# jhauret/vibravox

Measured on AMD Instinct MI355X. Metric: EBEN train-step audio-seconds/sec (gen+disc), higher is better.
Workload: dtype bf16

## Files before the change

vibravox_amd/csrc/bl_dw.hip:

```cpp
#include "common.h"

#include <cstdlib>

namespace eben {

typedef float f32x16 __attribute__((ext_vector_type(16)));
typedef __bf16 bf16x8 __attribute__((ext_vector_type(8)));
typedef short s16x4 __attribute__((ext_vector_type(4)));
typedef short s16x8 __attribute__((ext_vector_type(8)));
typedef unsigned u32x4 __attribute__((ext_vector_type(4)));

#ifndef EBEN_BLDW_DBG
#define EBEN_BLDW_DBG 0
#endif
#ifndef EBEN_BLDW_PIPE_FENCE
#define EBEN_BLDW_PIPE_FENCE 1
#endif
#ifdef EBEN_BLDW_STAMP
__device__ unsigned long long bldw_stamp[8192 * 8];
#define BLDW_T(v) const unsigned long long v = __builtin_amdgcn_s_memtime()
#endif
constexpr int BLDW_BKT = 64;
constexpr int BLDW_TS = 68;
constexpr int BLDW_RS_MAX = 132;
static int bldw_row_stride(int xneed) { int rs = xneed <= 4 ? 4 : xneed; while ((rs & 15) != 4) ++rs; return rs > BLDW_RS_MAX ? BLDW_RS_MAX : rs; }

struct BlDwArgs {
  const u32x4* ah; const u32x4* xh;
  float* slabs;
  int B, G, Mg, Cg, MgB, CgB, CBa, CBx, La, Lx;
  int S, d, k, pad, amin;
  int NQW;
  int has_bias, nnt, nmt, nsplit, nct, nchunks, XR, xneed;
  int dense, c_in_g, c_out_g, row_stride;
  int RS;
  int xw;
  long long slab_stride;
};

template <unsigned STEP4 = 64u>
__device__ __forceinline__ bf16x8 bl_tr_frag(unsigned addr) {
  typedef __attribute__((address_space(3))) s16x4* lds4_t;
  const s16x4 r0 = __builtin_amdgcn_ds_read_tr16_b64_v4i16((lds4_t)(size_t)(addr));
  const s16x4 r1 = __builtin_amdgcn_ds_read_tr16_b64_v4i16((lds4_t)(size_t)(addr + STEP4));
  const s16x8 v = {r0[0], r0[1], r0[2], r0[3], r1[0], r1[1], r1[2], r1[3]};
  return __builtin_bit_cast(bf16x8, v);
}

__device__ u32x4 bl_zero_unit = {0u, 0u, 0u, 0u};

__device__ __forceinline__ void bl_dma_piece(const u32x4* src, unsigned dst) {
  asm volatile("s_mov_b32 m0, %1\n\ts_nop 0\n\tglobal_load_lds_dwordx4 %0, off" :: "v"(src), "s"(dst) : "memory");
}

constexpr int BLDW_XC_S = 4;
template <int FM, int FN, bool XC = false, int WN = 2>
__device__ __forceinline__ void bl_dw_body(const BlDwArgs& P, unsigned bid, unsigned nblk) {
  constexpr int BM = 64 * FM, BMB = BM / 8, BNQ = 4 * WN * FN, BKT = BLDW_BKT, TS = BLDW_TS, NW = 2 * WN;
  const int RS = P.RS;
  extern __shared__ __attribute__((aligned(16))) u32x4 smem_bldw[];
  typedef __attribute__((address_space(3))) void* lds_t;
  const int tid = threadIdx.x, lane = tid & 63;
  const int wave = __builtin_amdgcn_readfirstlane(tid >> 6);
  const int wm = wave / WN, wn = wave % WN;

  unsigned id = xcd_remap(bid, nblk);
  const int z = __builtin_amdgcn_readfirstlane(id % P.nsplit); id /= P.nsplit;
  const int nti = __builtin_amdgcn_readfirstlane(id % P.nnt); id /= P.nnt;
  const int mt = __builtin_amdgcn_readfirstlane(id % P.nmt);
  const int g = __builtin_amdgcn_readfirstlane(id / P.nmt);

  const int q0 = nti * BNQ;
  int cb_lo = q0 / P.k;
  if (cb_lo > P.CgB - 1) cb_lo = P.CgB - 1;
  int qlast = q0 + BNQ < P.NQW ? q0 + BNQ : P.NQW;
  int cb_hi = (qlast - 1) / P.k;
  if (cb_hi < cb_lo) cb_hi = cb_lo;
  const int xrows = (cb_hi - cb_lo + 1) * (XC ? 1 : P.S);

  const int a_units = BMB * TS, buf_units = a_units + P.XR * RS;
  for (int i = tid; i < BLDW_TS; i += 64 * NW) smem_bldw[i] = u32x4{0x00003f80u, 0u, 0u, 0u};
  const unsigned lds0 = (unsigned)(unsigned long long)(lds_t)smem_bldw;
  const unsigned ones_addr = lds0, buf_addr = lds0 + BLDW_TS * 16;

  const int G4 = lane >> 4, js = (lane & 15) >> 2, qs = lane & 3;
  const int koff = 8 * (G4 >> 1) + js;
  unsigned aoff[FM], boff[FN];
  bool bconst[FN];
#pragma unroll
  for (int i = 0; i < FM; ++i) {
    const int bundle = (wm * FM + i) * 4 + 2 * (G4 & 1) + (qs >> 1);
    aoff[i] = (unsigned)((bundle * TS + koff) * 16 + 8 * (qs & 1));
  }
#pragma unroll
  for (int f = 0; f < FN; ++f) {
    const int q = q0 + 4 * (wn * FN + f) + 2 * (G4 & 1) + (qs >> 1);
    if (q < P.NQW) {
      const int cb = q / P.k, j = q - cb * P.k;
      const int off = j * P.d - P.pad;
      if (XC) {
        boff[f] = (unsigned)(a_units * 16 + ((cb - cb_lo) * RS + (off - P.amin * BLDW_XC_S) + koff * BLDW_XC_S) * 16 + 8 * (qs & 1));
      } else {
        int a = off / P.S;
        if (off < 0 && a * P.S != off) --a;
        const int p = off - a * P.S;
        const int row = (cb - cb_lo) * P.S + p;
        boff[f] = (unsigned)(a_units * 16 + (row * RS + (a - P.amin) + koff) * 16 + 8 * (qs & 1));
      }
      bconst[f] = false;
    } else {
      boff[f] = (unsigned)(koff * 16 + 8 * (qs & 1));
      bconst[f] = true;
    }
  }

  f32x16 acc[FM][FN];
#pragma unroll
  for (int i = 0; i < FM; ++i)
#pragma unroll
    for (int f = 0; f < FN; ++f)
#pragma unroll
      for (int r = 0; r < 16; ++r) acc[i][f][r] = 0.f;

  const u32x4* zero = &bl_zero_unit;
  constexpr int AR = (BMB + NW - 1) / NW;
  long long arow[AR];
#pragma unroll
  for (int i = 0; i < AR; ++i) {
    int bundle = g * P.MgB + mt * BMB + wave + NW * i;
    if (bundle > P.CBa - 1) bundle = P.CBa - 1;
    arow[i] = mt * BMB + wave + NW * i < P.MgB ? (long long)bundle * P.La : -1;
  }
  constexpr int XW = 4;
  const bool x_regs = XC || P.XR <= NW * XW;
  long long xoff[XW];
  int xlane[XW];
  unsigned xdst[XW];
  bool xact[XW];
  const int npr = XC ? (P.xw + 63) / 64 : 1;
#pragma unroll
  for (int i = 0; i < XW; ++i) {
    const int xr = wave + NW * i;
    if (XC) {
      const int row = xr / npr, pc = xr - row * npr;
      int cb = cb_lo + row;
      if (cb > P.CgB - 1) cb = P.CgB - 1;
      xoff[i] = ((long long)g * P.CgB + cb) * P.Lx;
      xlane[i] = P.amin * BLDW_XC_S + 64 * pc + lane;
      xdst[i] = (unsigned)((a_units + row * RS + 64 * pc) * 16);
      xact[i] = xr < xrows * npr && 64 * pc + lane < P.xw;
    } else {
      const int cbl = xr / P.S, p = xr - cbl * P.S;
      int cb = cb_lo + cbl;
      if (cb > P.CgB - 1) cb = P.CgB - 1;
      xoff[i] = ((long long)g * P.CgB + cb) * P.Lx;
      xlane[i] = (P.amin + lane) * P.S + p;
      xdst[i] = (unsigned)((a_units + xr * RS) * 16);
      xact[i] = true;
    }
  }
  const long long a_item = (long long)P.CBa * P.La, x_item = (long long)P.CBx * P.Lx;
  auto issue = [&](int b, int t0, int bsel) {
    const unsigned dst = buf_addr + (unsigned)(bsel * buf_units * 16);
    const u32x4* ab = P.ah + (long long)b * a_item + t0 + lane;
    const bool a_ok = t0 + lane < P.La;
#pragma unroll
    for (int i = 0; i < AR; ++i) {
      const int r = wave + NW * i;
      if (r < BMB && !(EBEN_BLDW_DBG & 1)) bl_dma_piece((a_ok && arow[i] >= 0) ? ab + arow[i] : zero, __builtin_amdgcn_readfirstlane(dst + (unsigned)(r * TS * 16)));
    }
    const u32x4* xb = P.xh + (long long)b * x_item;
    if (EBEN_BLDW_DBG & 2) return;
    if (XC) {
      const int ts = t0 * BLDW_XC_S;
#pragma unroll
      for (int i = 0; i < XW; ++i)
        if (wave + NW * i < xrows * npr) {
          const int pos0 = ts + xlane[i];
          if (xact[i]) bl_dma_piece((unsigned)pos0 < (unsigned)P.Lx ? xb + xoff[i] + pos0 : zero, __builtin_amdgcn_readfirstlane(dst + xdst[i]));
        }
      return;
    }
    if (x_regs) {
      const int ts = t0 * P.S;
#pragma unroll
      for (int i = 0; i < XW; ++i)
        if (wave + NW * i < xrows) {
          const u32x4* row = xb + xoff[i];
          const int pos0 = ts + xlane[i];
          const unsigned rdst = dst + xdst[i];
          bl_dma_piece((unsigned)pos0 < (unsigned)P.Lx ? row + pos0 : zero, __builtin_amdgcn_readfirstlane(rdst));
          if (64 + lane < P.xneed) {
            const int pos1 = pos0 + 64 * P.S;
            bl_dma_piece((unsigned)pos1 < (unsigned)P.Lx ? row + pos1 : zero, __builtin_amdgcn_readfirstlane(rdst + (unsigned)(64 * 16)));
          }
        }
      return;
    }
    for (int xr = wave; xr < xrows; xr += NW) {
      const int cbl = xr / P.S, p = xr - cbl * P.S;
      int cb = cb_lo + cbl;
      if (cb > P.CgB - 1) cb = P.CgB - 1;
      const u32x4* row = xb + ((long long)g * P.CgB + cb) * P.Lx;
      const unsigned rdst = dst + (unsigned)((a_units + xr * RS) * 16);
      const int pos0 = (t0 + P.amin + lane) * P.S + p;
      bl_dma_piece((pos0 >= 0 && pos0 < P.Lx) ? row + pos0 : zero, __builtin_amdgcn_readfirstlane(rdst));
      if (64 + lane < P.xneed) {
        const int pos1 = pos0 + 64 * P.S;
        bl_dma_piece((pos1 >= 0 && pos1 < P.Lx) ? row + pos1 : zero, __builtin_amdgcn_readfirstlane(rdst + (unsigned)(64 * 16)));
      }
    }
  };
  const int dq_b = P.nsplit / P.nct, dq_t = P.nsplit - dq_b * P.nct;
  int qb = z / P.nct, qt = z - qb * P.nct;

  int bsel = 0;
  auto advance = [&]() {
    qb += dq_b; qt += dq_t;
    if (qt >= P.nct) { qt -= P.nct; ++qb; }
  };
  if (z < P.nchunks) { issue(qb, qt * BKT, 0); advance(); }
#ifdef EBEN_BLDW_STAMP
  unsigned long long st_wait = 0, st_bar = 0, st_issue = 0, st_mma = 0, st_n = 0;
  const unsigned long long st_begin = __builtin_amdgcn_s_memtime();
#endif
  for (int q = z; q < P.nchunks; q += P.nsplit) {
#ifdef EBEN_BLDW_STAMP
    BLDW_T(ta);
#endif
    asm volatile("s_waitcnt vmcnt(0)" ::: "memory");
#ifdef EBEN_BLDW_STAMP
    BLDW_T(tb);
#endif
    __syncthreads();
#ifdef EBEN_BLDW_STAMP
    BLDW_T(tc);
#endif
    if (q + P.nsplit < P.nchunks) { issue(qb, qt * BKT, bsel ^ 1); advance(); }
#ifdef EBEN_BLDW_STAMP
    BLDW_T(td);
#endif
    const unsigned base = buf_addr + (unsigned)(bsel * buf_units * 16);
    constexpr unsigned BSTEP4 = XC ? 64u * BLDW_XC_S : 64u;
    bf16x8 av[2][FM], bv[2][FN];
#pragma unroll
    for (int i = 0; i < FM; ++i) av[0][i] = bl_tr_frag(base + aoff[i]);
#pragma unroll
    for (int f = 0; f < FN; ++f) bv[0][f] = bl_tr_frag<BSTEP4>(bconst[f] ? ones_addr + boff[f] : base + boff[f]);
#pragma unroll
    for (int ks = 0; ks < BKT / 16; ++ks) {
      const int cur = ks & 1, nxt = cur ^ 1;
      if (ks + 1 < BKT / 16) {
#pragma unroll
        for (int i = 0; i < FM; ++i) av[nxt][i] = bl_tr_frag(base + aoff[i] + (unsigned)((ks + 1) * 256));
#pragma unroll
        for (int f = 0; f < FN; ++f)
          bv[nxt][f] = bl_tr_frag<BSTEP4>(bconst[f] ? ones_addr + boff[f] : base + boff[f] + (unsigned)((ks + 1) * 4 * BSTEP4));
      }
#pragma unroll
      for (int i = 0; i < FM; ++i)
#pragma unroll
        for (int f = 0; f < FN; ++f) {
          if (EBEN_BLDW_DBG & 4) acc[i][f][0] += __builtin_bit_cast(float, __builtin_bit_cast(u32x4, av[cur][i])[0] ^ __builtin_bit_cast(u32x4, bv[cur][f])[1]);
          else acc[i][f] = __builtin_amdgcn_mfma_f32_32x32x16_bf16(av[cur][i], bv[cur][f], acc[i][f], 0, 0, 0);
        }
#if EBEN_BLDW_PIPE_FENCE
      __builtin_amdgcn_sched_barrier(0);
#endif
    }
    bsel ^= 1;
#ifdef EBEN_BLDW_STAMP
    { BLDW_T(te); st_wait += tb - ta; st_bar += tc - tb; st_issue += td - tc; st_mma += te - td; ++st_n; }
#endif
  }
#ifdef EBEN_BLDW_STAMP
  if (tid == 0 && bid < 8192u) {
    unsigned long long* o = bldw_stamp + bid * 8;
    o[0] = st_wait; o[1] = st_bar; o[2] = st_issue; o[3] = st_mma; o[4] = st_n; o[5] = __builtin_amdgcn_s_memtime() - st_begin;
  }
#endif

  float* slab = P.slabs + (long long)z * P.slab_stride;
  const int m_base = mt * BM + wm * FM * 32 + 4 * (lane >> 5);
#pragma unroll
  for (int f = 0; f < FN; ++f) {
    const int nl = lane & 31;
    const int q = q0 + 4 * (wn * FN + f) + (nl >> 3), e = nl & 7;
    long long col = -1;
    int cgrp = -1;
    if (!P.dense) {
      if (q < P.NQW || (q == P.NQW && e == 0 && P.has_bias)) col = 8LL * q + e;
    } else if (q < P.NQW) {
      const int cb = q / P.k, j = q - cb * P.k, c = 8 * cb + e;
      cgrp = c / P.c_in_g;
      col = (long long)(c - cgrp * P.c_in_g) * P.k + j;
    } else if (q == P.NQW && e == 0 && P.has_bias) {
      col = (long long)P.c_in_g * P.k;
    }
    if (col < 0) continue;
#pragma unroll
    for (int i = 0; i < FM; ++i)
#pragma unroll
      for (int r = 0; r < 16; ++r) {
        const int m = m_base + i * 32 + (r & 3) + 8 * (r >> 2);
        if (m >= P.Mg) continue;
        if (P.dense && cgrp >= 0 && m / P.c_out_g != cgrp) continue;
        if (!(EBEN_BLDW_DBG & 8) || acc[i][f][r] == 12345.f) slab[((long long)g * P.Mg + m) * P.row_stride + col] = acc[i][f][r];
      }
  }
}

template <int FM, int FN, bool XC = false, int WN = 2>
__global__ __launch_bounds__(128 * WN, 2) void bl_dw_kernel(const BlDwArgs P) { bl_dw_body<FM, FN, XC, WN>(P, blockIdx.x, gridDim.x); }

constexpr int BLDW_MULTI = 4;
struct BlDwTable {
  int n;
  unsigned first[BLDW_MULTI + 1];
  BlDwArgs job[BLDW_MULTI];
};
template <int FM, int FN>
__global__ __launch_bounds__(256, 2) void bl_dw_multi_kernel(const BlDwTable T) {
  int j = 0;
#pragma unroll 1
  while (j + 1 < T.n && blockIdx.x >= T.first[j + 1]) ++j;
  j = __builtin_amdgcn_readfirstlane(j);
  bl_dw_body<FM, FN>(T.job[j], blockIdx.x - T.first[j], T.first[j + 1] - T.first[j]);
}

struct BlDwPlan {
  int ok, G, Mg, Cg, MgB, CgB, dense, FM, FN, nmt, nnt, NQW, nct, nchunks, nsplit, XR, amin, row_stride, perm_k, xneed, RS, xc, xw, wide;
  size_t lds_bytes;
  long long slab_stride;
};

static int bldw_floordiv(int a, int b) { int q = a / b; if ((a % b != 0) && ((a < 0) != (b < 0))) --q; return q; }

static void make_bldw_plan(const Canon& c, BlDwPlan* p) {
  p->ok = 0;
  if (!c.bl || c.reflect || c.np != 1) return;
  p->G = c.g; p->Mg = c.Cout / c.g; p->Cg = c.Cin / c.g; p->dense = 0;
  if ((p->Mg & 7) || (p->Cg & 7)) { p->dense = 1; p->G = 1; p->Mg = c.Cout; p->Cg = c.Cin; }
  if ((p->Mg & 7) || (p->Cg & 7)) return;
  p->MgB = p->Mg / 8; p->CgB = p->Cg / 8;
  p->amin = bldw_floordiv(-c.pl, c.s);
  const int amax = bldw_floordiv((c.k - 1) * c.d - c.pl, c.s);
  if (amax - p->amin > 60 || c.s > 8) return;
  p->FM = (p->Mg > 64 && round_up(p->Mg, 128) == round_up(p->Mg, 64)) ? 2 : 1;
  p->NQW = p->CgB * c.k;
  static const int fn_max = getenv("EBEN_BLDW_FN") ? atoi(getenv("EBEN_BLDW_FN")) : 4;
  p->FN = (fn_max >= 4 && (c.k >= 16 || p->NQW >= 256)) ? 4 : p->NQW + 1 > 8 ? 2 : 1;
  static const int fn3_thin = getenv("EBEN_BLDW_FN3_THIN") ? atoi(getenv("EBEN_BLDW_FN3_THIN")) : 1;
  if (fn3_thin && p->FN == 2 && ceil_div(p->NQW + 1, 24) < ceil_div(p->NQW + 1, 16)) p->FN = 3;
  static const int fn3 = getenv("EBEN_BLDW_FN3") ? atoi(getenv("EBEN_BLDW_FN3")) : 1;
  if (fn3 && p->FN == 4 && p->FM == 2) {
    const int t4 = ceil_div(p->NQW + 1, 32) * ceil_div(p->Mg, 64 * p->FM) * p->G, t3 = ceil_div(p->NQW + 1, 24) * ceil_div(p->Mg, 64 * p->FM) * p->G;
    if (fn3 == 2 || (t4 <= 512 && t4 > 256 && t3 <= 512)) p->FN = 3;
  }
  static const int wide_on = getenv("EBEN_BLDW_WIDE") ? atoi(getenv("EBEN_BLDW_WIDE")) : 1;
  p->wide = (wide_on && p->FM == 2 && p->FN >= 3 && p->NQW + 1 >= 48 && c.s == BLDW_XC_S && c.d == 1) ? 1 : 0;
  if (p->wide) p->FN = 3;
  static const int xc_on = getenv("EBEN_BLDW_XC") ? atoi(getenv("EBEN_BLDW_XC")) : 1;
  p->nmt = ceil_div(p->Mg, 64 * p->FM);
  p->xneed = BLDW_BKT + amax - p->amin + 1;
  for (;;) {
    const int BNQ = (p->wide ? 16 : 8) * p->FN;
    p->nnt = ceil_div(p->NQW + 1, BNQ);
    int ncb = (BNQ - 1) / c.k + 2;
    if (ncb > p->CgB) ncb = p->CgB;
    p->XR = ncb * c.s;
    p->RS = bldw_row_stride(p->xneed);
    p->xc = 0; p->xw = 0;
    if (xc_on && c.s == BLDW_XC_S && c.d == 1 && p->FN >= 3) {
      const int xw = p->xneed * c.s;
      if (ncb * ceil_div(xw, 64) <= (p->wide ? 32 : 16)) {
        p->xc = 1; p->xw = xw; p->XR = ncb;
        p->RS = xw + 1;
      }
    }
    if (!p->wide || p->xc) break;
    p->wide = 0;
  }
  p->lds_bytes = 16ull * (BLDW_TS + 2ull * ((64 * p->FM / 8) * BLDW_TS + (unsigned long long)p->XR * p->RS));
  if (p->lds_bytes > 160 * 1024) return;
  p->nct = ceil_div(c.Lout, BLDW_BKT);
  p->nchunks = c.B * p->nct;
  const int tiles = p->nnt * p->nmt * p->G;
  static const int cus = getenv("EBEN_BLDW_CUS") ? atoi(getenv("EBEN_BLDW_CUS")) : 256;
  const int per_cu = p->wide ? 1 : (int)(160 * 1024 / p->lds_bytes) < 1 ? 1 : (int)(160 * 1024 / p->lds_bytes);
  const int slots = cus * (per_cu > 4 ? 4 : per_cu);
  const double macs = (double)c.B * c.Lout * (double)c.Cout * (c.Cin / c.g) * c.k;
  const double t_all = 2.0 * macs / 1.0e15;
  const double slab_bytes = 4.0 * (double)c.Cout * ((c.Cin / c.g) * c.k + 1);
  int ns = 1;
  double best = 1e30;
  for (int cand = 1; cand <= 256 && cand <= p->nchunks; ++cand) {
    const long long blocks = (long long)tiles * cand;
    const double rounds = (double)((blocks + slots - 1) / slots);
    const double t = rounds * (t_all * slots / blocks) + 2.0 * cand * slab_bytes / 2.0e12 + (cand > 1 ? slab_bytes / 2.0e12 + 5e-6 : 0.0);
    if (t < best * 0.97) { best = t; ns = cand; }
  }
  static const int force_ns = getenv("EBEN_BLDW_NSPLIT") ? atoi(getenv("EBEN_BLDW_NSPLIT")) : 0;
  if (force_ns > 0 && force_ns <= p->nchunks) ns = force_ns;
  p->nsplit = ns;
  if (p->dense) { p->row_stride = (c.Cin / c.g) * c.k + 1; p->perm_k = 0; }
  else { p->row_stride = p->Cg * c.k + 1; p->perm_k = c.k; }
  p->slab_stride = (long long)c.Cout * p->row_stride;
  p->ok = 1;
}

template <int FM, int FN, bool XC = false, int WN = 2>
static int launch_bldw(const BlDwArgs& a, const BlDwPlan& p, hipStream_t st) {
  static LdsAttrOnce attr_once;
  auto kern = bl_dw_kernel<FM, FN, XC, WN>;
  {
    const hipError_t e = lds_attr_once(attr_once, reinterpret_cast<const void*>(kern));
    if (e != hipSuccess) return hip_fail(e, "hipFuncSetAttribute(bl_dw)");
  }
  const long long nb = (long long)p.nnt * p.nmt * p.G * p.nsplit;
  hipLaunchKernelGGL(kern, dim3((unsigned)nb), dim3(128 * WN), p.lds_bytes, st, a);
  EBEN_CHECK_LAUNCH("bl_dw_kernel");
  return EBEN_OK;
}

struct BlDwVariant { int FM, FN, XC, WN, grouped; };
static BlDwVariant bldw_variant(const BlDwPlan& p) {
  if (p.wide) return BlDwVariant{2, 3, 1, 4, 0};
  return BlDwVariant{p.FM, p.FN, p.xc, 2, p.xc ? 0 : 1};
}

static int launch_bldw_variant(const BlDwVariant& v, const BlDwArgs& a, const BlDwPlan& p, hipStream_t st) {
  if (v.WN == 4) return launch_bldw<2, 3, true, 4>(a, p, st);
  if (v.XC) return v.FM == 2 ? (v.FN == 4 ? launch_bldw<2, 4, true>(a, p, st) : launch_bldw<2, 3, true>(a, p, st))
                             : (v.FN == 4 ? launch_bldw<1, 4, true>(a, p, st) : launch_bldw<1, 3, true>(a, p, st));
  if (v.FM == 2) return v.FN == 4 ? launch_bldw<2, 4>(a, p, st) : v.FN == 3 ? launch_bldw<2, 3>(a, p, st) : v.FN == 2 ? launch_bldw<2, 2>(a, p, st) : launch_bldw<2, 1>(a, p, st);
  return v.FN == 4 ? launch_bldw<1, 4>(a, p, st) : v.FN == 3 ? launch_bldw<1, 3>(a, p, st) : v.FN == 2 ? launch_bldw<1, 2>(a, p, st) : launch_bldw<1, 1>(a, p, st);
}

}

using namespace eben;

extern "C" size_t eben_bl_conv1d_bwd_dw_workspace(const EbenConv1dDesc* d, int* nslab, int* row_stride, int* col_perm_k) {
  Canon c;
  if (canon_from_desc(d, &c) != EBEN_OK || d->transposed) return 0;
  BlDwPlan p;
  make_bldw_plan(c, &p);
  if (!p.ok) return 0;
  if (nslab) *nslab = p.nsplit;
  if (row_stride) *row_stride = p.row_stride;
  if (col_perm_k) *col_perm_k = p.perm_k;
  return sizeof(float) * (size_t)p.slab_stride * p.nsplit;
}

static int bldw_args(const EbenConv1dDesc* d, const void* dy_hi, const void* x_hi, int has_bias, float* slabs, size_t ws_bytes, BlDwArgs* out,
                     BlDwPlan* plan) {
  Canon c;
  int rc = canon_from_desc(d, &c);
  if (rc) return rc;
  EBEN_REQUIRE(!d->transposed && dy_hi && x_hi && slabs, "eben_bl_conv1d_bwd_dw: a Conv1d descriptor and non-null operands");
  BlDwPlan p;
  make_bldw_plan(c, &p);
  if (!p.ok) return fail(EBEN_EUNSUPPORTED, "eben_bl_conv1d_bwd_dw: layer not covered by the bundle-layout weight-gradient kernel");
  const size_t need = sizeof(float) * (size_t)p.slab_stride * p.nsplit;
  if (ws_bytes < need) return fail(EBEN_EWORKSPACE, "bl bwd_dw needs %zu workspace bytes, got %zu", need, ws_bytes);
  BlDwArgs a;
  a.ah = static_cast<const u32x4*>(dy_hi); a.xh = static_cast<const u32x4*>(x_hi); a.slabs = slabs;
  a.B = c.B; a.G = p.G; a.Mg = p.Mg; a.Cg = p.Cg; a.MgB = p.MgB; a.CgB = p.CgB; a.CBa = c.Cout / 8; a.CBx = c.Cin / 8; a.La = c.Lout; a.Lx = c.Lin;
  a.S = c.s; a.d = c.d; a.k = c.k; a.pad = c.pl; a.amin = p.amin; a.NQW = p.NQW; a.has_bias = has_bias ? 1 : 0;
  a.nnt = p.nnt; a.nmt = p.nmt; a.nsplit = p.nsplit; a.nct = p.nct; a.nchunks = p.nchunks; a.XR = p.XR;
  a.dense = p.dense; a.c_in_g = c.Cin / c.g; a.c_out_g = c.Cout / c.g; a.row_stride = p.row_stride; a.slab_stride = p.slab_stride;
  a.xneed = p.xneed; a.RS = p.RS; a.xw = p.xw;
  *out = a; *plan = p;
  return EBEN_OK;
}

extern "C" int eben_bl_conv1d_bwd_dw(const EbenConv1dDesc* d, const void* dy_hi, const void* x_hi, int has_bias, float* slabs, size_t ws_bytes,
                                     void* stream) {
  BlDwArgs a;
  BlDwPlan p;
  const int rc = bldw_args(d, dy_hi, x_hi, has_bias, slabs, ws_bytes, &a, &p);
  if (rc) return rc;
  return launch_bldw_variant(bldw_variant(p), a, p, as_stream(stream));
}

extern "C" int eben_bl_conv1d_bwd_dw_variant(const EbenConv1dDesc* d, int* out, int n) {
  EBEN_REQUIRE(out && n >= 5, "eben_bl_conv1d_bwd_dw_variant: 5 output slots");
  Canon c;
  const int rc = canon_from_desc(d, &c);
  if (rc) return rc;
  EBEN_REQUIRE(!d->transposed, "eben_bl_conv1d_bwd_dw_variant: a Conv1d descriptor");
  BlDwPlan p;
  make_bldw_plan(c, &p);
  if (!p.ok) return fail(EBEN_EUNSUPPORTED, "eben_bl_conv1d_bwd_dw_variant: layer not covered by the bundle-layout weight-gradient kernel");
  const BlDwVariant v = bldw_variant(p);
  out[0] = v.FM; out[1] = v.FN; out[2] = v.XC; out[3] = v.WN; out[4] = v.grouped;
  return EBEN_OK;
}

namespace eben {
template <int FM, int FN>
static int launch_bldw_multi(const BlDwTable& T, size_t lds, hipStream_t st) {
  static LdsAttrOnce attr_once;
  auto kern = bl_dw_multi_kernel<FM, FN>;
  {
    const hipError_t e = lds_attr_once(attr_once, reinterpret_cast<const void*>(kern));
    if (e != hipSuccess) return hip_fail(e, "hipFuncSetAttribute(bl_dw_multi)");
  }
  hipLaunchKernelGGL(kern, dim3(T.first[T.n]), dim3(256), lds, st, T);
  EBEN_CHECK_LAUNCH("bl_dw_multi_kernel");
  return EBEN_OK;
}
}

extern "C" int eben_bl_conv1d_bwd_dw_multi(const EbenConv1dDesc* const* descs, const void* const* dy_hi, const void* const* x_hi, int has_bias,
                                           float* const* slabs, const size_t* ws_bytes, int n, void* stream) {
  EBEN_REQUIRE(descs && dy_hi && x_hi && slabs && ws_bytes && n > 0, "bad eben_bl_conv1d_bwd_dw_multi arguments");
  hipStream_t st = as_stream(stream);
  int i = 0;
  while (i < n) {
    BlDwTable T;
    T.n = 0; T.first[0] = 0;
    BlDwPlan p0{};
    size_t lds = 0;
    while (i < n && T.n < BLDW_MULTI) {
      BlDwArgs a;
      BlDwPlan p;
      const int rc = bldw_args(descs[i], dy_hi[i], x_hi[i], has_bias, slabs[i], ws_bytes[i], &a, &p);
      if (rc) return rc;
      if (!bldw_variant(p).grouped) {
        if (T.n > 0) break;
        const int rc1 = eben_bl_conv1d_bwd_dw(descs[i], dy_hi[i], x_hi[i], has_bias, slabs[i], ws_bytes[i], stream);
        if (rc1) return rc1;
        ++i;
        continue;
      }
      if (T.n > 0 && (p.FM != p0.FM || p.FN != p0.FN)) break;
      const long long nb = (long long)p.nnt * p.nmt * p.G * p.nsplit;
      if (nb <= 0 || nb > 0x3fffffffLL - (long long)T.first[T.n]) return fail(EBEN_EINVAL, "bl bwd_dw_multi grid too large");
      if (T.n == 0) p0 = p;
      T.job[T.n] = a;
      T.first[T.n + 1] = T.first[T.n] + (unsigned)nb;
      if (p.lds_bytes > lds) lds = p.lds_bytes;
      ++T.n; ++i;
    }
    if (T.n == 0) continue;
    int rc;
    if (p0.FM == 2) rc = p0.FN == 4 ? launch_bldw_multi<2, 4>(T, lds, st) : p0.FN == 3 ? launch_bldw_multi<2, 3>(T, lds, st) : p0.FN == 2 ? launch_bldw_multi<2, 2>(T, lds, st) : launch_bldw_multi<2, 1>(T, lds, st);
    else rc = p0.FN == 4 ? launch_bldw_multi<1, 4>(T, lds, st) : p0.FN == 3 ? launch_bldw_multi<1, 3>(T, lds, st) : p0.FN == 2 ? launch_bldw_multi<1, 2>(T, lds, st) : launch_bldw_multi<1, 1>(T, lds, st);
    if (rc) return rc;
  }
  return EBEN_OK;
}

#ifdef EBEN_BLDW_STAMP
extern "C" __attribute__((visibility("default"))) int eben_debug_bldw_stamps(unsigned long long* out, size_t n) {
  return (int)hipMemcpyFromSymbol(out, HIP_SYMBOL(eben::bldw_stamp), n * sizeof(unsigned long long));
}
#endif
```

Measured before the change: 7387.

## Add thin weight-gradient kernel with multi-stage LDS ring and contiguous chunk ranges

Adds a THIN variant of the bundle-layout weight-gradient kernel for layers with few output tiles and many K chunks. Each block takes a contiguous range of chunks and runs a 3-deep (2 for XC) LDS ring, waiting with partial vmcnt counts so loads stay in flight across iterations instead of draining to zero every step. Block count is sized to the CU count, so fewer split slabs are reduced later. The trade-offs are more LDS per block, fewer resident blocks and lower occupancy, and a new set of tuning environment variables.

```diff
diff --git a/vibravox_amd/csrc/bl_dw.hip b/vibravox_amd/csrc/bl_dw.hip
--- a/vibravox_amd/csrc/bl_dw.hip
+++ b/vibravox_amd/csrc/bl_dw.hip
@@ -22,6 +22,8 @@
 #endif
 constexpr int BLDW_BKT = 64;
 constexpr int BLDW_TS = 68;
+constexpr int BLDW_THIN_RING = 3, BLDW_THIN_RING_XC = 2;
+constexpr int BLDW_THIN_PER_CU = 1, BLDW_THIN_PER_CU_XC = 3;
 constexpr int BLDW_RS_MAX = 132;
 static int bldw_row_stride(int xneed) { int rs = xneed <= 4 ? 4 : xneed; while ((rs & 15) != 4) ++rs; return rs > BLDW_RS_MAX ? BLDW_RS_MAX : rs; }
 
@@ -35,6 +37,7 @@
   int dense, c_in_g, c_out_g, row_stride;
   int RS;
   int xw;
+  int cpb;
   long long slab_stride;
 };
 
@@ -54,7 +57,17 @@
 }
 
 constexpr int BLDW_XC_S = 4;
-template <int FM, int FN, bool XC = false, int WN = 2>
+__device__ __forceinline__ void bl_wait_pieces(int n) {
+#define BLDW_VM(k) case k: asm volatile("s_waitcnt vmcnt(" #k ")" ::: "memory"); break;
+  switch (n) {
+    BLDW_VM(1) BLDW_VM(2) BLDW_VM(3) BLDW_VM(4) BLDW_VM(5) BLDW_VM(6) BLDW_VM(7) BLDW_VM(8) BLDW_VM(9) BLDW_VM(10)
+    BLDW_VM(11) BLDW_VM(12) BLDW_VM(13) BLDW_VM(14) BLDW_VM(15) BLDW_VM(16) BLDW_VM(17) BLDW_VM(18) BLDW_VM(19) BLDW_VM(20)
+    default: asm volatile("s_waitcnt vmcnt(0)" ::: "memory"); break;
+  }
+#undef BLDW_VM
+}
+
+template <int FM, int FN, bool XC = false, int WN = 2, bool THIN = false, int RING = 2>
 __device__ __forceinline__ void bl_dw_body(const BlDwArgs& P, unsigned bid, unsigned nblk) {
   constexpr int BM = 64 * FM, BMB = BM / 8, BNQ = 4 * WN * FN, BKT = BLDW_BKT, TS = BLDW_TS, NW = 2 * WN;
   const int RS = P.RS;
@@ -211,36 +224,7 @@
       }
     }
   };
-  const int dq_b = P.nsplit / P.nct, dq_t = P.nsplit - dq_b * P.nct;
-  int qb = z / P.nct, qt = z - qb * P.nct;
-
-  int bsel = 0;
-  auto advance = [&]() {
-    qb += dq_b; qt += dq_t;
-    if (qt >= P.nct) { qt -= P.nct; ++qb; }
-  };
-  if (z < P.nchunks) { issue(qb, qt * BKT, 0); advance(); }
-#ifdef EBEN_BLDW_STAMP
-  unsigned long long st_wait = 0, st_bar = 0, st_issue = 0, st_mma = 0, st_n = 0;
-  const unsigned long long st_begin = __builtin_amdgcn_s_memtime();
-#endif
-  for (int q = z; q < P.nchunks; q += P.nsplit) {
-#ifdef EBEN_BLDW_STAMP
-    BLDW_T(ta);
-#endif
-    asm volatile("s_waitcnt vmcnt(0)" ::: "memory");
-#ifdef EBEN_BLDW_STAMP
-    BLDW_T(tb);
-#endif
-    __syncthreads();
-#ifdef EBEN_BLDW_STAMP
-    BLDW_T(tc);
-#endif
-    if (q + P.nsplit < P.nchunks) { issue(qb, qt * BKT, bsel ^ 1); advance(); }
-#ifdef EBEN_BLDW_STAMP
-    BLDW_T(td);
-#endif
-    const unsigned base = buf_addr + (unsigned)(bsel * buf_units * 16);
+  auto mma_chunk = [&](const unsigned base) {
     constexpr unsigned BSTEP4 = XC ? 64u * BLDW_XC_S : 64u;
     bf16x8 av[2][FM], bv[2][FN];
 #pragma unroll
@@ -268,17 +252,75 @@
       __builtin_amdgcn_sched_barrier(0);
 #endif
     }
-    bsel ^= 1;
-#ifdef EBEN_BLDW_STAMP
-    { BLDW_T(te); st_wait += tb - ta; st_bar += tc - tb; st_issue += td - tc; st_mma += te - td; ++st_n; }
-#endif
-  }
-#ifdef EBEN_BLDW_STAMP
-  if (tid == 0 && bid < 8192u) {
-    unsigned long long* o = bldw_stamp + bid * 8;
-    o[0] = st_wait; o[1] = st_bar; o[2] = st_issue; o[3] = st_mma; o[4] = st_n; o[5] = __builtin_amdgcn_s_memtime() - st_begin;
-  }
-#endif
+  };
+  if constexpr (THIN) {
+    int n_w = AR;
+#pragma unroll
+    for (int i = 0; i < XW; ++i)
+      if (wave + NW * i < xrows * npr) n_w += XC ? 1 : 2;
+    n_w = __builtin_amdgcn_readfirstlane(n_w);
+    const int first = z * P.cpb;
+    int n_my = P.nchunks - first;
+    if (n_my > P.cpb) n_my = P.cpb;
+    int qb = first / P.nct, qt = first - qb * P.nct;
+    auto advance = [&]() { if (++qt == P.nct) { qt = 0; ++qb; } };
+    int issued = 0;
+    for (; issued < RING - 1 && issued < n_my; ++issued) { issue(qb, qt * BKT, issued); advance(); }
+    int slot = 0, islot = RING - 1;
+    for (int i = 0; i < n_my; ++i) {
+      if (issued - 1 - i >= RING - 2) bl_wait_pieces((RING - 2) * n_w);
+      else asm volatile("s_waitcnt vmcnt(0)" ::: "memory");
+      __syncthreads();
+      if (issued < n_my) {
+        issue(qb, qt * BKT, islot); advance(); ++issued;
+        islot = islot + 1 == RING ? 0 : islot + 1;
+      }
+      mma_chunk(buf_addr + (unsigned)(slot * buf_units * 16));
+      slot = slot + 1 == RING ? 0 : slot + 1;
+    }
+  } else {
+    const int dq_b = P.nsplit / P.nct, dq_t = P.nsplit - dq_b * P.nct;
+    int qb = z / P.nct, qt = z - qb * P.nct;
+
+    int bsel = 0;
+    auto advance = [&]() {
+      qb += dq_b; qt += dq_t;
+      if (qt >= P.nct) { qt -= P.nct; ++qb; }
+    };
+    if (z < P.nchunks) { issue(qb, qt * BKT, 0); advance(); }
+#ifdef EBEN_BLDW_STAMP
+    unsigned long long st_wait = 0, st_bar = 0, st_issue = 0, st_mma = 0, st_n = 0;
+    const unsigned long long st_begin = __builtin_amdgcn_s_memtime();
+#endif
+    for (int q = z; q < P.nchunks; q += P.nsplit) {
+#ifdef EBEN_BLDW_STAMP
+      BLDW_T(ta);
+#endif
+      asm volatile("s_waitcnt vmcnt(0)" ::: "memory");
+#ifdef EBEN_BLDW_STAMP
+      BLDW_T(tb);
+#endif
+      __syncthreads();
+#ifdef EBEN_BLDW_STAMP
+      BLDW_T(tc);
+#endif
+      if (q + P.nsplit < P.nchunks) { issue(qb, qt * BKT, bsel ^ 1); advance(); }
+#ifdef EBEN_BLDW_STAMP
+      BLDW_T(td);
+#endif
+      mma_chunk(buf_addr + (unsigned)(bsel * buf_units * 16));
+      bsel ^= 1;
+#ifdef EBEN_BLDW_STAMP
+      { BLDW_T(te); st_wait += tb - ta; st_bar += tc - tb; st_issue += td - tc; st_mma += te - td; ++st_n; }
+#endif
+    }
+#ifdef EBEN_BLDW_STAMP
+    if (tid == 0 && bid < 8192u) {
+      unsigned long long* o = bldw_stamp + bid * 8;
+      o[0] = st_wait; o[1] = st_bar; o[2] = st_issue; o[3] = st_mma; o[4] = st_n; o[5] = __builtin_amdgcn_s_memtime() - st_begin;
+    }
+#endif
+  }
 
   float* slab = P.slabs + (long long)z * P.slab_stride;
   const int m_base = mt * BM + wm * FM * 32 + 4 * (lane >> 5);
@@ -304,7 +346,9 @@
       for (int r = 0; r < 16; ++r) {
         const int m = m_base + i * 32 + (r & 3) + 8 * (r >> 2);
         if (m >= P.Mg) continue;
-        if (P.dense && cgrp >= 0 && m / P.c_out_g != cgrp) continue;
+        if (THIN) {
+          if (P.dense && cgrp >= 0 && (unsigned)(m - cgrp * P.c_out_g) >= (unsigned)P.c_out_g) continue;
+        } else if (P.dense && cgrp >= 0 && m / P.c_out_g != cgrp) continue;
         if (!(EBEN_BLDW_DBG & 8) || acc[i][f][r] == 12345.f) slab[((long long)g * P.Mg + m) * P.row_stride + col] = acc[i][f][r];
       }
   }
@@ -312,6 +356,9 @@
 
 template <int FM, int FN, bool XC = false, int WN = 2>
 __global__ __launch_bounds__(128 * WN, 2) void bl_dw_kernel(const BlDwArgs P) { bl_dw_body<FM, FN, XC, WN>(P, blockIdx.x, gridDim.x); }
+
+template <int FM, int FN, bool XC, int RING>
+__global__ __launch_bounds__(256, 2) void bl_dw_thin_kernel(const BlDwArgs P) { bl_dw_body<FM, FN, XC, 2, true, RING>(P, blockIdx.x, gridDim.x); }
 
 constexpr int BLDW_MULTI = 4;
 struct BlDwTable {
@@ -330,6 +377,7 @@
 
 struct BlDwPlan {
   int ok, G, Mg, Cg, MgB, CgB, dense, FM, FN, nmt, nnt, NQW, nct, nchunks, nsplit, XR, amin, row_stride, perm_k, xneed, RS, xc, xw, wide;
+  int thin, ring, cpb;
   size_t lds_bytes;
   long long slab_stride;
 };
@@ -403,6 +451,30 @@
   static const int force_ns = getenv("EBEN_BLDW_NSPLIT") ? atoi(getenv("EBEN_BLDW_NSPLIT")) : 0;
   if (force_ns > 0 && force_ns <= p->nchunks) ns = force_ns;
   p->nsplit = ns;
+  static const int thin_on = getenv("EBEN_THIN_DW") ? atoi(getenv("EBEN_THIN_DW")) : 1;
+  static const int thin_xc = getenv("EBEN_THIN_DW_XC") ? atoi(getenv("EBEN_THIN_DW_XC")) : 1;
+  static const int ring_s2 = getenv("EBEN_THIN_DW_RING") ? atoi(getenv("EBEN_THIN_DW_RING")) : BLDW_THIN_RING;
+  static const int ring_xc = getenv("EBEN_THIN_DW_RING_XC") ? atoi(getenv("EBEN_THIN_DW_RING_XC")) : BLDW_THIN_RING_XC;
+  static const int blocks_s2 = getenv("EBEN_THIN_DW_BLOCKS") ? atoi(getenv("EBEN_THIN_DW_BLOCKS")) : 0;
+  static const int blocks_xc = getenv("EBEN_THIN_DW_BLOCKS_XC") ? atoi(getenv("EBEN_THIN_DW_BLOCKS_XC")) : 0;
+  const int thin_ring = p->xc ? ring_xc : ring_s2, thin_blocks = p->xc ? blocks_xc : blocks_s2;
+  p->thin = 0; p->ring = 2; p->cpb = 0;
+  const bool thin_shape = !p->wide && ((p->FN == 3 && !p->xc) || (p->FN == 4 && p->xc && thin_xc)) && (p->xc || p->XR <= 16);
+  if (thin_on && thin_shape && tiles <= 24 && p->nchunks >= 512 && thin_ring >= 2 && thin_ring <= 4) {
+    const size_t lds = 16ull * (BLDW_TS + (unsigned long long)thin_ring * ((64 * p->FM / 8) * BLDW_TS + (unsigned long long)p->XR * p->RS));
+    if (lds <= 160 * 1024) {
+      const int fit = (int)(160 * 1024 / lds);
+      const int per_cu = p->xc ? BLDW_THIN_PER_CU_XC : BLDW_THIN_PER_CU;
+      const int want = thin_blocks > 0 ? thin_blocks : cus * (fit > per_cu || p->xc ? per_cu : fit);
+      int nz = want / tiles;
+      if (nz < 1) nz = 1;
+      int cpb = ceil_div(p->nchunks, nz);
+      if (cpb < thin_ring) cpb = thin_ring;
+      p->thin = 1; p->ring = thin_ring; p->cpb = cpb;
+      p->nsplit = ceil_div(p->nchunks, cpb);
+      p->lds_bytes = lds;
+    }
+  }
   if (p->dense) { p->row_stride = (c.Cin / c.g) * c.k + 1; p->perm_k = 0; }
   else { p->row_stride = p->Cg * c.k + 1; p->perm_k = c.k; }
   p->slab_stride = (long long)c.Cout * p->row_stride;
@@ -426,10 +498,33 @@
 struct BlDwVariant { int FM, FN, XC, WN, grouped; };
 static BlDwVariant bldw_variant(const BlDwPlan& p) {
   if (p.wide) return BlDwVariant{2, 3, 1, 4, 0};
-  return BlDwVariant{p.FM, p.FN, p.xc, 2, p.xc ? 0 : 1};
+  return BlDwVariant{p.FM, p.FN, p.xc, 2, (p.xc || p.thin) ? 0 : 1};
+}
+
+template <int FM, int FN, bool XC, int RING>
+static int launch_bldw_thin(const BlDwArgs& a, const BlDwPlan& p, hipStream_t st) {
+  static LdsAttrOnce attr_once;
+  auto kern = bl_dw_thin_kernel<FM, FN, XC, RING>;
+  {
+    const hipError_t e = lds_attr_once(attr_once, reinterpret_cast<const void*>(kern));
+    if (e != hipSuccess) return hip_fail(e, "hipFuncSetAttribute(bl_dw_thin)");
+  }
+  const long long nb = (long long)p.nnt * p.nmt * p.G * p.nsplit;
+  hipLaunchKernelGGL(kern, dim3((unsigned)nb), dim3(256), p.lds_bytes, st, a);
+  EBEN_CHECK_LAUNCH("bl_dw_thin_kernel");
+  return EBEN_OK;
+}
+
+template <int FM, int FN, bool XC>
+static int launch_bldw_thin_ring(const BlDwArgs& a, const BlDwPlan& p, hipStream_t st) {
+  return p.ring == 2 ? launch_bldw_thin<FM, FN, XC, 2>(a, p, st) : p.ring == 3 ? launch_bldw_thin<FM, FN, XC, 3>(a, p, st) : launch_bldw_thin<FM, FN, XC, 4>(a, p, st);
 }
 
 static int launch_bldw_variant(const BlDwVariant& v, const BlDwArgs& a, const BlDwPlan& p, hipStream_t st) {
+  if (p.thin) {
+    if (v.XC) return v.FM == 2 ? launch_bldw_thin_ring<2, 4, true>(a, p, st) : launch_bldw_thin_ring<1, 4, true>(a, p, st);
+    return v.FM == 2 ? launch_bldw_thin_ring<2, 3, false>(a, p, st) : launch_bldw_thin_ring<1, 3, false>(a, p, st);
+  }
   if (v.WN == 4) return launch_bldw<2, 3, true, 4>(a, p, st);
   if (v.XC) return v.FM == 2 ? (v.FN == 4 ? launch_bldw<2, 4, true>(a, p, st) : launch_bldw<2, 3, true>(a, p, st))
                              : (v.FN == 4 ? launch_bldw<1, 4, true>(a, p, st) : launch_bldw<1, 3, true>(a, p, st));
@@ -470,7 +565,7 @@
   a.S = c.s; a.d = c.d; a.k = c.k; a.pad = c.pl; a.amin = p.amin; a.NQW = p.NQW; a.has_bias = has_bias ? 1 : 0;
   a.nnt = p.nnt; a.nmt = p.nmt; a.nsplit = p.nsplit; a.nct = p.nct; a.nchunks = p.nchunks; a.XR = p.XR;
   a.dense = p.dense; a.c_in_g = c.Cin / c.g; a.c_out_g = c.Cout / c.g; a.row_stride = p.row_stride; a.slab_stride = p.slab_stride;
-  a.xneed = p.xneed; a.RS = p.RS; a.xw = p.xw;
+  a.xneed = p.xneed; a.RS = p.RS; a.xw = p.xw; a.cpb = p.cpb;
   *out = a; *plan = p;
   return EBEN_OK;
 }
```

After: 7336. Within noise of the previous version (-0.7%).
